# Mikubill/sketch2img

Measured on AMD Instinct MI355X. Metric: sketch-guided images/sec whole-node, SD1.5 512px 50-step DDIM, higher is better.
Workload: dtype fp16

## Files before the change

include/skg.h:

```cpp
#ifndef SKG_H_
#define SKG_H_

#include <stddef.h>
#include <stdint.h>

#ifdef __cplusplus
extern "C" {
#endif

#define SKG_OK 0
#define SKG_E_BADARG (-1)
#define SKG_E_UNSUPPORTED (-2)
#define SKG_E_LAUNCH (-3)

#define SKG_ABI_VERSION 6
int skg_abi_version(void);
const char* skg_last_error(void);

#define SKG_EPI_RELU 1u
#define SKG_EPI_OUT_F32 2u
#define SKG_EPI_GEGLU 4u
#define SKG_EPI_BIAS_ROWS 8u

int skg_gemm_f16(const void* A, int lda, const void* B, int ldb, void* C, void* C_lo, int ldc, int M, int N, int K,
                 const void* bias, const void* residual, const void* residual_lo, int ldr, float alpha, unsigned flags,
                 float* gn_partial, int HW, int groups, void* stream);

int skg_set_workspace(void* ws, size_t bytes, void* stream);

int skg_gemm_variant(int M, int N, int K, int Cin, int mode);

#define SKG_CONV_S1 0
#define SKG_CONV_S2 1
#define SKG_CONV_UP2 2
#define SKG_CONV_S2T 3
#define SKG_CONV_S2A 4
int skg_conv3x3_f16(const void* X, int ldx, const void* Wp, void* Y, void* Y_lo, int ldy, int rows, int IH, int IW,
                    int Cin, int Cout, int mode, const void* bias, const void* residual, const void* residual_lo, int ldr,
                    float alpha, unsigned flags, float* gn_partial, int groups, void* stream);

size_t skg_groupnorm_scratch_floats(int rows, int groups);
int skg_groupnorm_stats(const void* X, int ldx, int rows, int HW, int C, int groups, float eps,
                        float* stats, float* partial, void* stream);
int skg_groupnorm_fwd(const void* X, const void* X_lo, int ldx, void* Y, void* Y_lo, int ldy, int rows, int HW, int C, int groups,
                      float eps, const void* gamma, const void* beta, int silu, float* stats, float* partial, void* stream);
// ... 180 lines not shown
```

sketch2img_amd/_lib.py:

```python
from __future__ import annotations

import ctypes
import os

import torch

_HERE = os.path.dirname(os.path.abspath(__file__))
LIB_PATH = os.environ.get("SKG_LIB") or os.path.join(_HERE, "libskg.so")

ABI_VERSION = 6

SIGNATURES = {
    "skg_abi_version": ("i", ""),
    "skg_last_error": ("s", ""),
    "skg_gemm_f16": ("i", "pipippiiiipppifupiip"),
    "skg_conv3x3_up2_f16": ("i", "pipppiiiiiiipp"),
    "skg_conv3x3_sc_f16": ("i", "pipiipppiiiiiipupip"),
    "skg_conv4x4s2_f16": ("i", "pippiiiiiipp"),
    "skg_conv3x3_wino_v_bytes": ("z", "iiii"),
    "skg_conv3x3_wino_f16": ("i", "pippppiiiiiipppiup"),
    "skg_groupnorm_wino_fwd": ("i", "pipiiiiifppipp"),
    "skg_gemm_f16_rows": ("i", "pipipiiiipiip"),
    "skg_gemm_gn_fused": ("i", "iiiiiii"),
    "skg_gemm_f16_geglu_keep": ("i", "pipipipiiiipp"),
    "skg_ff_block_f16": ("i", "ppippiiiippfppppppippiipiip"),
    "skg_xattn_block_f16": ("i", "ppippiiiiiippfpppfpppipip"),
    "skg_gemm_variant": ("i", "iiiii"),
    "skg_set_workspace": ("i", "pzp"),
    "skg_conv3x3_f16": ("i", "pipppiiiiiiipppifupip"),
    "skg_groupnorm_scratch_floats": ("z", "ii"),
    "skg_groupnorm_stats": ("i", "piiiiifppp"),
    "skg_groupnorm_fwd": ("i", "ppippiiiiifppippp"),
    "skg_groupnorm_from_partial": ("i", "ppippiiiiiifppippipiip"),
    "skg_groupnorm_apply": ("i", "ppipiiiiipppip"),
    "skg_groupnorm_bwd": ("i", "pipipipiiiiipppipp"),
    "skg_layernorm_fwd": ("i", "ppipiiippfpp"),
    "skg_layernorm_bwd": ("i", "pipipipiiippp"),
    "skg_geglu_fwd": ("i", "pipiiiip"),
    "skg_geglu_bwd": ("i", "pipipiiiip"),
    "skg_attn_fwd": ("i", "pipipipipiiiiiifup"),
    "skg_attn_bwd_delta": ("i", "pipipiiiip"),
    "skg_attn_bwd_dq": ("i", "pipipipipippppiiiiiiifp"),
# ... 94 lines not shown
```

sketch2img_amd/csrc/gemm.hip:

```cpp
#include "gemm_params.h"
#include <mutex>
#include <vector>

namespace {

constexpr int BM = 128;
constexpr int BK = 32;
constexpr int PITCH = 40;

template <int BN, int MODE>
__global__ __launch_bounds__(256) void gemm_kernel(const GemmParams p) {
  constexpr int WN = BN / 2;
  constexpr int NT = WN / 16;
  constexpr int MT = 4;
  constexpr int BPT = BN / 64;
  __shared__ __attribute__((aligned(16))) half_t As[2][BM * PITCH];
  __shared__ __attribute__((aligned(16))) half_t Bs[2][BN * PITCH];

  const int tid = threadIdx.x;
  const int lane = tid & 63;
  const int wave = tid >> 6;
  const int wm = wave >> 1, wn = wave & 1;
  const int g = lane >> 4, l16 = lane & 15;
  const int m0 = blockIdx.y * BM;
// ... 266 lines not shown
#ifdef SKG_LAB
    q.C = (void*)16;
    if (skg_gemm9_eligible(q, mode)) return 9320;
    q.C = nullptr;
#endif
    if (const int bn8 = skg_gemm8_tile_n(q, mode)) return 8000 + bn8;
#ifdef SKG_LAB
    q.C = (void*)16;
    if (skg_gemmk_eligible(q, mode)) return 9160;
#endif
  }
  const int v2 = skg_gemm2_tile_n(M, N, K, Cin, mode, ws_query_bytes());
  return v2 ? 2000 + v2 : 1000 + (use_wide(M, N) ? 128 : 64);
}

extern "C" int skg_gemm_f16_geglu_keep(const void* A, int lda, const void* B, int ldb, void* Y, int ldy, void* H,
                                       int ldh, int M, int N, int K, const void* bias, void* stream) {
  SKG_REQUIRE(A && B && Y && H && M > 0 && N > 0 && K > 0 && K % 64 == 0 && N % 16 == 0);
  SKG_REQUIRE(lda % 8 == 0 && ldb % 8 == 0 && ldy % 8 == 0 && ldh % 8 == 0 && lda >= K && ldb >= K && ldy >= N / 2 && ldh >= N);
  SKG_REQUIRE(skg_aligned(A, 16) && skg_aligned(B, 16) && skg_aligned(Y, 16) && skg_aligned(H, 16));
  SKG_REQUIRE(!bias || skg_aligned(bias, 8));
  GemmParams p{};
  p.A = (const half_t*)A; p.lda = lda; p.B = (const half_t*)B; p.ldb = ldb; p.C = Y; p.ldc = ldy;
  p.bias = (const half_t*)bias; p.M = M; p.N = N; p.K = K; p.alpha = 1.f; p.flags = SKG_EPI_GEGLU;
  p.aux = (half_t*)H; p.ldaux = ldh;
  ws_attach(p, (hipStream_t)stream);
  return launch<MODE_DIRECT>(p, (hipStream_t)stream);
}

extern "C" int skg_gemm_gn_fused(int M, int N, int K, int Cin, int mode, int HW, int groups) {
// ... 227 lines not shown
```

sketch2img_amd/csrc/gemm2.hip:

```cpp
#include "gemm_params.h"
#include <stdlib.h>

namespace {

constexpr int BK = 64;
constexpr unsigned OOB = 0x80000000u;

typedef __attribute__((address_space(3))) void* lds_ptr_t;

__device__ __forceinline__ void dma16(__amdgpu_buffer_rsrc_t rsrc, half_t* lds_wave_base, unsigned voff,
                                      unsigned soff) {
  __builtin_amdgcn_raw_ptr_buffer_load_lds(rsrc, (lds_ptr_t)lds_wave_base, 16, voff, soff, 0, 0);
}

template <int MASK, int N>
__device__ __forceinline__ void sgb() {
  if constexpr (N > 0) __builtin_amdgcn_sched_group_barrier(MASK, N, 0);
}
constexpr int SGB_MFMA = 0x008, SGB_VMEM = 0x010, SGB_DSREAD = 0x100;
template <int NT, int R, int V>
__device__ __forceinline__ void sched_group() {
  if constexpr (NT > 0) {
    sgb<SGB_MFMA, 1>();
    if constexpr (R > 0) {
// ... 82 lines not shown
  if (p.flags & SKG_EPI_RELU) {
    v[0] = fmaxf(v[0], 0.f); v[1] = fmaxf(v[1], 0.f); v[2] = fmaxf(v[2], 0.f); v[3] = fmaxf(v[3], 0.f);
  }
  if (p.flags & SKG_EPI_OUT_F32) {
    *reinterpret_cast<float4_t*>(reinterpret_cast<float*>(p.C) + m * p.ldc + n) = v;
  } else {
    half4_t o = {(half_t)v[0], (half_t)v[1], (half_t)v[2], (half_t)v[3]};
    st_half4(reinterpret_cast<half_t*>(p.C) + m * p.ldc + n, o);
    if (p.c_lo) {
      half4_t l = {(half_t)(v[0] - (float)o[0]), (half_t)(v[1] - (float)o[1]), (half_t)(v[2] - (float)o[2]), (half_t)(v[3] - (float)o[3])};
      st_half4(p.c_lo + m * p.ldc + n, l);
    }
  }
}

template <int BM, int BN, int WGM, int WGN, int MODE, int NS, bool GNS, bool HILO, bool FIX, bool BROWS = false>
__device__ __forceinline__ void gemm2_body(const GemmParams& p, int tiles_n, int nwg, unsigned a_bytes, unsigned b_bytes,
                                           unsigned a_shift, int kt_per_split, float* __restrict__ ws) {
  constexpr int NW = WGM * WGN;
  constexpr int NTHR = NW * 64;
  constexpr int WM = BM / WGM;
  constexpr int WN = BN / WGN;
  constexpr int NT = WN / 16;
  constexpr int MT = WM / 16;
  constexpr int ACH = BM / 8 / NW;
  constexpr int BCH = BN / 8 / NW;
  static_assert(BM % (8 * NW) == 0 && BN % (8 * NW) == 0 && WM % 16 == 0 && WN % 16 == 0, "tile shape");
  constexpr int STAGE = (BM + BN) * BK;
  constexpr bool AFFINE = (MODE == MODE_DIRECT || MODE == MODE_S1 || MODE == MODE_S2 || MODE == MODE_S2A);
  __shared__ __attribute__((aligned(16))) half_t smem[NS * STAGE + 2 * BN];

  const int tid = threadIdx.x;
  const int lane = tid & 63;
  const int wave = __builtin_amdgcn_readfirstlane(tid >> 6);
  const int wm = wave / WGN, wn = wave - wm * WGN;
  const int g = lane >> 4, l16 = lane & 15;

  const __amdgpu_buffer_rsrc_t rA =
      __builtin_amdgcn_make_buffer_rsrc((void*)((const char*)p.A - a_shift), 0, a_bytes, 0x00020000);
  const __amdgpu_buffer_rsrc_t rB = __builtin_amdgcn_make_buffer_rsrc((void*)p.B, 0, b_bytes, 0x00020000);
  const __amdgpu_buffer_rsrc_t rA2 = __builtin_amdgcn_make_buffer_rsrc(
      (void*)(p.A2 ? p.A2 : p.A), 0, p.A2 ? ((unsigned)(p.M - 1) * (unsigned)p.lda2 + (unsigned)p.K2) * 2u : 0u, 0x00020000);
  const int KT1 = (MODE == MODE_S1 && p.K2) ? (p.K - p.K2) / BK : (1 << 30);

  for (int vb = blockIdx.x; vb < nwg; vb += gridDim.x) {
// ... 80 lines not shown
      } else {
        a_voff[j] = ok ? 0u : OOB;
        a_oy[j] = oy; a_ox[j] = ox;
        a_img[j] = img * (unsigned)p.lda * 2u + pk + a_shift;
      }
    }
  }
  unsigned b_voff[BCH];
#pragma unroll
  for (int j = 0; j < BCH; ++j) {
    const int r = (j * NW + wave) * 8 + lr;
    const unsigned pk = (unsigned)(lq ^ ((r >> 1) & 7)) * 16u;
    const int n = n0 + r;
    b_voff[j] = n < p.N ? ((unsigned)n + (p.up2 == 5 ? (unsigned)(ph * p.N) : 0u)) * (unsigned)p.ldb * 2u + pk : OOB;
  }

  const bool tap_minor = (p.flags & 0x1000u) != 0;
  struct DmaStep { unsigned va[ACH]; unsigned vb[BCH]; unsigned soa, sob; bool second; };
  auto dma_prepare = [&](int kt, bool live) {
    DmaStep d;
    d.second = false;
    if (MODE == MODE_S1 && kt >= KT1) {
      d.second = true;
#pragma unroll
      for (int j = 0; j < ACH; ++j) {
        const int r = (j * NW + wave) * 8 + lr;
        const unsigned pk = (unsigned)(lq ^ ((r >> 1) & 7)) * 16u;
        d.va[j] = (live && m0 + r < p.M) ? (unsigned)(m0 + r) * (unsigned)p.lda2 * 2u + pk : OOB;
      }
#pragma unroll
// ... 154 lines not shown
#ifdef SKG_LAB
    if (!(p.flags & 0x2000u))
#endif
    sched_plan<MT, NT, ND>();
  };

  const int kt_begin = split * kt_per_split;
  const int KT = min(p.K / BK, kt_begin + kt_per_split);
  float bias_r = 0.f;
  if constexpr (!BROWS) {
    const half_t* bias_t = p.bias;
    if constexpr (MODE != MODE_DIRECT) bias_t += __builtin_amdgcn_readfirstlane(smp0) * p.bias_pitch;
    bias_r = (tid < BN && p.bias && n0 + tid < p.N) ? (float)bias_t[n0 + tid] : 0.f;
  }
  SKG_PH(1);
  {
    const DmaStep d0 = dma_prepare(kt_begin, true);
#pragma unroll
    for (int i = 0; i < ND; ++i) dma_one(d0, 0, i);
  }
  if constexpr (NS == 2) {
    for (int kt = kt_begin; kt < KT; kt += 2) {
      asm volatile("s_waitcnt vmcnt(0)" ::: "memory");
      lds_barrier();
      step(kt + 1, 1, 0, KT);
      if (kt + 1 < KT) {
        asm volatile("s_waitcnt vmcnt(0)" ::: "memory");
        lds_barrier();
        step(kt + 2, 0, 1, KT);
      }
    }
  } else {
    static_assert(NS >= 3 && (NS - 2) * ND <= 63, "counted wait");
#pragma unroll
    for (int s = 1; s < NS - 1; ++s) {
      const DmaStep d1 = dma_prepare(kt_begin + s, kt_begin + s < KT);
#pragma unroll
      for (int i = 0; i < ND; ++i) dma_one(d1, s, i);
    }
    asm volatile("s_waitcnt vmcnt(0)" ::: "memory");
    for (int kt = kt_begin; kt < KT; kt += NS) {
#pragma unroll
      for (int s = 0; s < NS; ++s) {
        if (kt + s < KT) {
          asm volatile("s_waitcnt vmcnt(%0)" ::"n"((NS - 2) * ND) : "memory");
          lds_barrier();
          step(kt + s + NS - 1, (s + NS - 1) % NS, s, KT);
        }
      }
    }
  }
  asm volatile("s_waitcnt vmcnt(0)" ::: "memory");

  SKG_PH(2);
#ifdef SKG_PHASES
  if ((tid & 63) == 0 && vb < (1 << 15)) g_phase[vb][12 + (tid >> 6)] = __builtin_readcyclecounter();
#endif
  const bool stream_out = p.flags & 0x800u;
  const bool relu = p.flags & SKG_EPI_RELU;
  const bool f32out = p.flags & SKG_EPI_OUT_F32;
  if (ws) {
    float* slab = ws + (size_t)split * p.M * p.N;
#pragma unroll
    for (int i = 0; i < MT; ++i) {
      const int m = m0 + wm * WM + i * 16 + l16;
// ... 146 lines not shown
        const int nch = p.gn_hw >> 7, b = m0 / p.gn_hw, chunk = (m0 - b * p.gn_hw) >> 7;
        p.gn_partial[(((size_t)b * nch + chunk) * p.gn_groups + n0 / cpg + gi) * 2 + qq] = t;
      }
    }
  };
  if (staged && !p.res && !HILO && !BROWS) {
    constexpr int OPH = BN + 8;
    constexpr int HROWS = 128;
    constexpr int HSLABS = BM / HROWS;
    constexpr int PPR = BN / 8;
    constexpr int TPR2 = NTHR / 64;
    constexpr int IT2 = PPR / TPR2;
    constexpr int RPT = HROWS / 64;
    static_assert(HROWS * OPH * 2 <= 2 * STAGE * 2 && NTHR % 64 == 0 && PPR % TPR2 == 0, "fp16 staging slab");
    half_t* const hst = smem;
    float* const bias_s = reinterpret_cast<float*>(smem + NS * STAGE);
    const int er = tid / TPR2, ec = (tid % TPR2) * 8;
    const bool geglu = p.flags & SKG_EPI_GEGLU;
    if (tid < BN) bias_s[tid] = bias_r;
    half_t* const crow0 = reinterpret_cast<half_t*>(p.C) + (size_t)(m0 + er) * p.ldc + n0 + ec;
#pragma unroll
    for (int sl = 0; sl < HSLABS; ++sl) {
      lds_barrier();
      if (sl == 0) SKG_PH(8);
      if (WM < HROWS || wm == sl) {
#pragma unroll
        for (int j = 0; j < NT; ++j) {
          const float4_t b4 = *reinterpret_cast<const float4_t*>(&bias_s[wn * WN + j * 16 + g * 4]) * p.alpha;
#pragma unroll
          for (int i = 0; i < MT; ++i) acc[i][j] = acc[i][j] * p.alpha + b4;
        }
// ... 101 lines not shown
    }
    if (gn) gn_fold();
    SKG_PH(4);
    continue;
  }
  if (staged) {
    constexpr int OPF = BN + 4;
    constexpr int SROWS = 64;
    constexpr int SLABS = BM / SROWS;
    static_assert(SROWS * OPF * 4 <= 2 * STAGE * 2, "staging slab must fit in the pipeline stages");
    constexpr int PPR = BN / 8;
    constexpr int TPR = NTHR / SROWS;
    constexpr int ITER = PPR / TPR;
    static_assert(NTHR % SROWS == 0 && PPR % TPR == 0, "piece loop must have a compile-time trip count");
    float* const stg = reinterpret_cast<float*>(smem);
    float* const bias_s = reinterpret_cast<float*>(smem + NS * STAGE);
    const int er = tid / TPR, ec = (tid % TPR) * 8;
    if (tid < BN) bias_s[tid] = bias_r;
    constexpr bool RES_UP_FRONT = SLABS * ITER <= 10;
    half8_t rv[SLABS][ITER];
    const half_t* const rrow0 = p.res ? p.res + (size_t)(m0 + er) * p.ldr + n0 + ec : nullptr;
    auto load_res = [&](int sl) {
      const bool rowok = p.res && m0 + sl * SROWS + er < p.M;
#pragma unroll
      for (int k = 0; k < ITER; ++k)
        rv[sl][k] = (rowok && n0 + ec + k * TPR * 8 < p.N)
                        ? ld_half8(rrow0 + (size_t)sl * SROWS * p.ldr + k * TPR * 8) : zero_half8();
    };
    if (RES_UP_FRONT) {
#pragma unroll
      for (int sl = 0; sl < SLABS; ++sl) load_res(sl);
// ... 121 lines not shown
      }
      if (relu) {
        v[0] = fmaxf(v[0], 0.f); v[1] = fmaxf(v[1], 0.f); v[2] = fmaxf(v[2], 0.f); v[3] = fmaxf(v[3], 0.f);
      }
      if (f32out) {
        *reinterpret_cast<float4_t*>(reinterpret_cast<float*>(p.C) + (size_t)m * p.ldc + n) = v;
      } else {
        half4_t o = {(half_t)v[0], (half_t)v[1], (half_t)v[2], (half_t)v[3]};
        st_half4(reinterpret_cast<half_t*>(p.C) + (size_t)m * p.ldc + n, o);
      }
    }
  }
  }
}

template <int BM, int BN, int WGM, int WGN, int MODE, int NS = 2, bool GNS = false, bool HILO = false, bool BROWS = false>
__global__ __launch_bounds__(WGM * WGN * 64, (NS * (BM + BN) * BK * 2 + 8 * BN <= 80 * 1024) ? 2 : 1) void gemm2_kernel(const GemmParams p, int tiles_n, int nwg,
                                                                  unsigned a_bytes, unsigned b_bytes,
                                                                  unsigned a_shift, int kt_per_split,
                                                                  float* __restrict__ ws) {
  gemm2_body<BM, BN, WGM, WGN, MODE, NS, GNS, HILO, false, BROWS>(p, tiles_n, nwg, a_bytes, b_bytes, a_shift, kt_per_split, ws);
}
#ifdef SKG_LAB
template <int BM, int BN, int WGM, int WGN, int MODE>
__global__ __launch_bounds__(WGM * WGN * 64, (2 * (BM + BN) * BK * 2 + 8 * BN <= 80 * 1024) ? 2 : 1) void gemm2_splitk_kernel(const GemmParams p, int tiles_n, int nwg,
                                                                  unsigned a_bytes, unsigned b_bytes,
                                                                  unsigned a_shift, int kt_per_split,
                                                                  float* __restrict__ ws) {
  gemm2_body<BM, BN, WGM, WGN, MODE, 2, false, false, true>(p, tiles_n, nwg, a_bytes, b_bytes, a_shift, kt_per_split, ws);
}
#endif

__global__ __launch_bounds__(256) void splitk_reduce_kernel(const GemmParams p, const float* __restrict__ ws,
                                                            int splits) {
  const int N4 = p.N >> 2;
  const size_t total = (size_t)p.M * N4;
// ... 86 lines not shown

inline bool gn_fusable(const GemmParams& p, int mode) {
  if (!p.gn_partial || p.gn_groups <= 0 || p.gn_hw <= 0 || !eligible(p, mode)) return false;
  if (p.flags & (SKG_EPI_OUT_F32 | SKG_EPI_GEGLU)) return false;
  const bool hilo = p.c_lo || p.res_lo;
  TileCfg t = pick_tile(p.M, p.N, p.K);
  if (hilo && t.bm == 256) t = TileCfg{128, 160};
  if (t.bm != 128 || t.bn != 160) return false;
  if (p.M % 128 != 0 || p.N % 160 != 0 || p.gn_hw % 128 != 0 || p.M % p.gn_hw != 0 || p.N % p.gn_groups != 0) return false;
  const int cpg = p.N / p.gn_groups;
  if ((cpg & 1) || 160 % cpg != 0) return false;
  if (p.ldc % 8 != 0 || (reinterpret_cast<uintptr_t>(p.C) & 15) != 0) return false;
  if (p.res && (p.ldr % 8 != 0 || (reinterpret_cast<uintptr_t>(p.res) & 15) != 0)) return false;
  const long ntiles = (long)(p.M / 128) * (p.N / 160);
  return pick_splits(ntiles, p.K / BK, (size_t)p.M * p.N * 4, p.ws, p.ws_bytes) == 1;
}

template <int BM, int BN, int WGM, int WGN, int MODE>
void launch_cfg(const GemmParams& p_in, hipStream_t st) {
  GemmParams p = p_in;
  const size_t out_bytes = (size_t)p.M * ((p.flags & SKG_EPI_GEGLU) ? p.N / 2 : p.N) * ((p.flags & SKG_EPI_OUT_F32) ? 4 : 2);
  static const bool tap_major = getenv("SKG_TAP_MAJOR") != nullptr;
  if (MODE != MODE_DIRECT && !tap_major) p.flags |= 0x1000u;
#ifdef SKG_LAB
  if (MODE != MODE_DIRECT && getenv("SKG_GLUE_PROBE")) p.flags |= 0x2000u;
#endif
  static const char* smb = getenv("SKG_STREAM_MB");
  if (out_bytes >= (smb ? (size_t)atoi(smb) << 20 : STREAM_OUT_BYTES)) p.flags |= 0x800u;
#ifdef SKG_LAB
  static const int direct_epi = getenv("SKG_DIRECT_EPI") ? atoi(getenv("SKG_DIRECT_EPI")) : 0;
  const bool direct_ok = direct_epi && !(p.flags & (SKG_EPI_GEGLU | SKG_EPI_OUT_F32)) && !p.c_lo && !p.res_lo && !p.gn_partial && !p.up2 &&
                         !p.seg_rows && !p.ntaps && !p.bias_pitch && p.N % BN == 0 && p.ldc % 8 == 0 && skg_aligned(p.C, 16) &&
                         (!p.res || (p.ldr % 8 == 0 && skg_aligned(p.res, 16))) && (!p.bias || skg_aligned(p.bias, 16)) &&
                         (direct_epi == 1 || p.K <= 640);
#else
  constexpr bool direct_ok = false;
#endif
  const int tiles_n = skg_cdiv(p.N, BN);
  const int ntiles = skg_cdiv(p.M, BM) * tiles_n * (p.up2 == 5 ? 4 : 1);
  unsigned long long a, b, s;
  operand_bytes(p, MODE, a, b, s);
  const int KT = p.K / BK;
  int splits = (BM == 128 && !(p.flags & SKG_EPI_GEGLU) && !p.up2 && !p.seg_rows) ? pick_splits(ntiles, KT, (size_t)p.M * p.N * 4, p.ws, p.ws_bytes) : 1;
  if (p.wino) splits = p.wino;
  constexpr int NTHR = WGM * WGN * 64;
  if (BM == 128 && BN == 160 && splits == 1 && gn_fusable(p, MODE)) p.flags |= SKG_FLAG_GN_STATS;
  if (p.bias_pitch && (p.gn_hw % BM != 0 || (p.flags & SKG_EPI_OUT_F32) || p.ldc % 8 != 0 || !skg_aligned(p.C, 16) || (p.res && (p.ldr % 8 != 0 || !skg_aligned(p.res, 16)))))
    p.flags |= SKG_FLAG_BIAS_PER_ROW;
  if (direct_ok && splits == 1) p.flags |= 0x10000u;
  const int ns_eff = splits > 1 ? skg_cdiv(KT, skg_cdiv(KT, splits)) : 1;
  const int G = (8 % ns_eff == 0) ? 8 / ns_eff : 0;
  if (G >= 2 && ntiles % G == 0 && p.up2 != 5) {
    static const bool off = getenv("SKG_NO_XGRID") != nullptr;
    const int tiles_m = ntiles / tiles_n;
    const double a_mb = (double)p.M * (MODE == MODE_DIRECT ? p.K : p.Cin) * 2.0, w_mb = (double)p.N * p.K * 2.0;
    int best = 1;
    double cost = a_mb + G * w_mb;
    for (int gn = 2; gn <= G; gn *= 2) {
      if (tiles_n % gn != 0 || tiles_m % (G / gn) != 0) continue;
      const double c = gn * a_mb + (G / gn) * w_mb;
      if (c < 0.9 * cost) { cost = c; best = gn; }
    }
    static const char* force_gn = getenv("SKG_XGRID_GN");
// ... 9 lines not shown
#ifdef SKG_LAB
    if constexpr (BM == 128) {
      const bool self = getenv("SKG_SPLITK_SELF") != nullptr;
      if (p.ws_cnt && self && (size_t)ntiles * 4 <= SKG_WS_TICKET_BYTES && p.N % 4 == 0) {
        hipLaunchKernelGGL((gemm2_splitk_kernel<BM, BN, WGM, WGN, MODE>), dim3(ntiles * ns), dim3(NTHR), 0, st, p, tiles_n, ntiles * ns,
                           (unsigned)a, (unsigned)b, (unsigned)s, per, p.ws);
        return;
      }
    }
#endif
    bool deep = false;
    if constexpr (BM == 128 && BN == 160 && (MODE == MODE_DIRECT || MODE == MODE_S1)) {
      const int sns = split_tuning().ns;
      if (ntiles * ns <= 256 && per >= 4 && sns >= 3) {
        deep = true;
        if (sns >= 4)
          hipLaunchKernelGGL((gemm2_kernel<BM, BN, WGM, WGN, MODE, 4, false, false>), dim3(ntiles * ns), dim3(NTHR), 0, st, p, tiles_n, ntiles * ns,
                             (unsigned)a, (unsigned)b, (unsigned)s, per, p.ws);
        else
          hipLaunchKernelGGL((gemm2_kernel<BM, BN, WGM, WGN, MODE, 3, false, false>), dim3(ntiles * ns), dim3(NTHR), 0, st, p, tiles_n, ntiles * ns,
                             (unsigned)a, (unsigned)b, (unsigned)s, per, p.ws);
      }
    }
    if (!deep)
      hipLaunchKernelGGL((gemm2_kernel<BM, BN, WGM, WGN, MODE>), dim3(persistent_grid(ntiles * ns, NTHR)), dim3(NTHR),
                         0, st, p, tiles_n, ntiles * ns, (unsigned)a, (unsigned)b, (unsigned)s, per, p.ws);
    if (p.wino) return;
    size_t blocks = ((size_t)p.M * (p.N / 4) + 255) / 256;
    hipLaunchKernelGGL(splitk_reduce_kernel, dim3((unsigned)(blocks > 2048 ? 2048 : blocks)), dim3(256), 0, st, p,
                       (const float*)p.ws, ns);
    return;
// ... 18 lines not shown
#define G2_LAUNCH(NS_, GNS_, HILO_)                                                                                            \
  hipLaunchKernelGGL((gemm2_kernel<BM, BN, WGM, WGN, MODE, NS_, GNS_, HILO_>), dim3(ntiles), dim3(NTHR), 0, st, p, tiles_n, ntiles, \
                     (unsigned)a, (unsigned)b, (unsigned)s, KT, (float*)nullptr)
  if constexpr (BM == 128 && (BN == 160 || BN == 64) && (MODE == MODE_DIRECT || MODE == MODE_S1)) {
    static const bool off = getenv("SKG_NO_NS3") != nullptr;
#ifdef SKG_LAB
    if (!off && !gns && !hilo && ntiles <= 256) {
      const char* e = getenv("SKG_NS");
      const int ns = e ? atoi(e) : 0;
      if (ns == 4 && KT >= 5) { G2_LAUNCH(4, false, false); return; }
      if constexpr (BN == 64) {
        if (ns == 6 && KT >= 7) { G2_LAUNCH(6, false, false); return; }
      }
    }
#endif
    if (!off && KT >= 4 && (BN == 64 || ntiles <= 256)) {
      if constexpr (BN == 160) {
        if (gns) {
          if (hilo) G2_LAUNCH(3, true, true); else G2_LAUNCH(3, true, false);
          return;
        }
      }
      if (hilo) G2_LAUNCH(3, false, true); else G2_LAUNCH(3, false, false);
      return;
    }
  }
#ifdef SKG_PHASES
  static const char* solo = getenv("SKG_SOLO");
  if (solo) {
    hipLaunchKernelGGL((gemm2_kernel<BM, BN, WGM, WGN, MODE>), dim3(ntiles), dim3(NTHR), 48 * 1024, st,
                       p, tiles_n, ntiles, (unsigned)a, (unsigned)b, (unsigned)s, KT, (float*)nullptr);
// ... 10 lines not shown
    }
  }
  if constexpr (BM == 128 && BN == 160) {
    if (gns) { G2_LAUNCH(2, true, false); return; }
  }
#undef G2_LAUNCH
  hipLaunchKernelGGL((gemm2_kernel<BM, BN, WGM, WGN, MODE>), dim3(persistent_grid(ntiles, NTHR)), dim3(NTHR), 0, st,
                     p, tiles_n, ntiles, (unsigned)a, (unsigned)b, (unsigned)s, KT, (float*)nullptr);
}

template <int MODE>
void launch_mode(const GemmParams& p, hipStream_t st) {
  TileCfg t = pick_tile(p.M, p.N, p.K);
  if (t.bm == 256 && (p.c_lo || p.res_lo || p.up2 || p.seg_rows || p.bias_pitch)) t = TileCfg{128, 160};
  if (p.wino) t = p.N % 160 == 0 ? TileCfg{128, 160} : p.N % 128 == 0 ? TileCfg{128, 128} : TileCfg{128, 64};
  if (t.bm == 256) launch_cfg<256, 320, 2, 4, MODE>(p, st);
  else if (t.bn == 160) {
    launch_cfg<128, 160, 2, 2, MODE>(p, st);
  }
  else if (t.bn == 128) launch_cfg<128, 128, 2, 2, MODE>(p, st);
  else launch_cfg<128, 64, 2, 2, MODE>(p, st);
}

}

int skg_gemm2_tile_n(int M, int N, int K, int Cin, int mode, size_t ws_bytes) {
  if (K % BK != 0 || M < 1 || (mode != MODE_DIRECT && Cin % BK != 0)) return 0;
  const TileCfg t = pick_tile(M, N, K);
  const int KT = K / BK;
  const long ntiles = (long)skg_cdiv(M, t.bm) * skg_cdiv(N, t.bn);
  const int splits = t.bm == 128 ? pick_splits(ntiles, KT, (size_t)M * N * 4, ws_bytes ? (const float*)1 : nullptr, ws_bytes) : 1;
  bool three = t.bm == 128 && (t.bn == 160 || t.bn == 64) && (mode == MODE_DIRECT || mode == MODE_S1) &&
               !getenv("SKG_NO_NS3") && KT >= 4 && (t.bn == 64 || ntiles <= 256) && splits == 1;
  if (splits > 1 && t.bm == 128 && t.bn == 160 && (mode == MODE_DIRECT || mode == MODE_S1)) {
    const int per = skg_cdiv(KT, splits), ns = skg_cdiv(KT, per);
    three = ntiles * ns <= 256 && per >= 4 && split_tuning().ns >= 3;
  }
  return t.bn + (three ? 10000 : 0);
}

bool skg_gemm2_fuses_gn(const GemmParams& p, int mode) { return gn_fusable(p, mode); }

void skg_splitk_reduce_launch(const GemmParams& p, const float* ws, int splits, hipStream_t st) {
  size_t blocks = ((size_t)p.M * (p.N / 4) + 255) / 256;
  hipLaunchKernelGGL(splitk_reduce_kernel, dim3((unsigned)(blocks > 2048 ? 2048 : blocks)), dim3(256), 0, st, p, ws, splits);
}

bool skg_gemm2_try_launch(const GemmParams& p, int mode, hipStream_t st) {
  if (!eligible(p, mode)) return false;
  if (p.wino &&
      (mode != MODE_DIRECT || p.wino != 16 || (p.K / BK) % 16 != 0 || !p.ws || (size_t)16 * p.M * p.N * 4 > p.ws_bytes || p.gn_partial ||
       p.seg_rows || p.up2 || p.aux || (p.flags & (SKG_EPI_GEGLU | SKG_EPI_OUT_F32))))
    return false;
  if (p.seg_rows &&
      (mode != MODE_DIRECT || p.res || p.gn_partial || p.c_lo || p.res_lo || p.aux || (p.flags & (SKG_EPI_GEGLU | SKG_EPI_OUT_F32)) ||
       p.ldc % 8 != 0 || (reinterpret_cast<uintptr_t>(p.C) & 15) != 0))
// ... 33 lines not shown
```

sketch2img_amd/csrc/gemm_params.h:

```cpp
#pragma once
#include "common.h"

enum { MODE_DIRECT = 0, MODE_S1 = 1, MODE_S2 = 2, MODE_UP2 = 3, MODE_S2T = 4, MODE_S2A = 5 };

struct GemmParams {
  const half_t* A; int lda;
  const half_t* B; int ldb;
  void* C; int ldc;
  const half_t* bias;
  const half_t* res; int ldr;
  int M, N, K;
  float alpha; unsigned flags;
  int IH, IW, OH, OW, Cin;
  float* gn_partial; int gn_hw, gn_groups;
  half_t* aux; int ldaux;
  const half_t* res_lo; half_t* c_lo;
  int ntaps; unsigned tapmap; int up2;
  int a_wrap;
  int seg_rows, seg_stride;
  const half_t* A2; int lda2, K2;
  int wino;
  float* ws; size_t ws_bytes;
  unsigned* ws_cnt;
  int bias_pitch;
};
constexpr unsigned SKG_FLAG_GN_STATS = 0x8000u;
constexpr unsigned SKG_FLAG_BIAS_PER_ROW = 0x20000u;

bool skg_gemm2_try_launch(const GemmParams& p, int mode, hipStream_t st);
constexpr size_t SKG_WS_TICKET_BYTES = 16 << 10;
int skg_gemm2_tile_n(int M, int N, int K, int Cin, int mode, size_t ws_bytes);
bool skg_gemmws_eligible(const GemmParams& p, int mode);
bool skg_gemmws_try_launch(const GemmParams& p, int mode, hipStream_t st);
bool skg_gemm8_eligible(const GemmParams& p, int mode);
int skg_gemm8_tile_n(const GemmParams& p, int mode);
bool skg_gemm8_try_launch(const GemmParams& p, int mode, hipStream_t st);
bool skg_gemm9_eligible(const GemmParams& p, int mode);
bool skg_gemm9_try_launch(const GemmParams& p, int mode, hipStream_t st);
bool skg_gemmk_eligible(const GemmParams& p, int mode);
bool skg_gemmk_try_launch(const GemmParams& p, int mode, hipStream_t st);
void skg_splitk_reduce_launch(const GemmParams& p, const float* ws, int splits, hipStream_t st);
bool skg_gemm8_fuses_gn(const GemmParams& p, int mode);
bool skg_gemm2_fuses_gn(const GemmParams& p, int mode);
void skg_wino_in_launch(const half_t* X, int ldx, half_t* V, int rows, int IH, int IW, int Cin, hipStream_t st);
void skg_wino_out_launch(const GemmParams& p, const float* slabs, int IH, int IW, hipStream_t st);
void skg_gn_partial_launch(const half_t* X, int ldx, int rows, int HW, int C, int groups, int nch, float* partial,
// ... 2 lines not shown
```

Measured before the change: 6.136.

## Add halo-slab implicit-GEMM path for stride-1 3x3 convs

Adds a slab variant of the 128x160 gemm2 kernel for stride-1 3x3 convolutions. It loads a haloed input slab (rows plus a one-pixel border) into LDS once per channel block and reuses it across all nine taps, instead of re-gathering the A operand for each tap. Slab loads are double-buffered, and weight tiles go through a three-stage ring. The path is enabled by default at level 2 and selected by shape and split heuristics, with an env var and API to change the level. The cost is more LDS per block, more precomputed address registers and much more kernel complexity, with a risk of lower occupancy.

New measurement: 6.196, median of 6. No clear change (+1.0%).

```diff
diff --git a/include/skg.h b/include/skg.h
--- a/include/skg.h
+++ b/include/skg.h
@@ -29,6 +29,9 @@
 int skg_set_workspace(void* ws, size_t bytes, void* stream);
 
 int skg_gemm_variant(int M, int N, int K, int Cin, int mode);
+
+int skg_conv_slab_set(int level);
+int skg_conv_slab_takes(int rows, int IH, int IW, int Cin, int Cout, int K2, int pair);
 
 #define SKG_CONV_S1 0
 #define SKG_CONV_S2 1
diff --git a/sketch2img_amd/_lib.py b/sketch2img_amd/_lib.py
--- a/sketch2img_amd/_lib.py
+++ b/sketch2img_amd/_lib.py
@@ -26,6 +26,8 @@
     "skg_ff_block_f16": ("i", "ppippiiiippfppppppippiipiip"),
     "skg_xattn_block_f16": ("i", "ppippiiiiiippfpppfpppipip"),
     "skg_gemm_variant": ("i", "iiiii"),
+    "skg_conv_slab_set": ("i", "i"),
+    "skg_conv_slab_takes": ("i", "iiiiiii"),
     "skg_set_workspace": ("i", "pzp"),
     "skg_conv3x3_f16": ("i", "pipppiiiiiiipppifupip"),
     "skg_groupnorm_scratch_floats": ("z", "ii"),
diff --git a/sketch2img_amd/csrc/gemm.hip b/sketch2img_amd/csrc/gemm.hip
--- a/sketch2img_amd/csrc/gemm.hip
+++ b/sketch2img_amd/csrc/gemm.hip
@@ -304,6 +304,21 @@
   return v2 ? 2000 + v2 : 1000 + (use_wide(M, N) ? 128 : 64);
 }
 
+extern "C" int skg_conv_slab_set(int level) { return skg_gemm2_conv_slab_set(level); }
+
+extern "C" int skg_conv_slab_takes(int rows, int IH, int IW, int Cin, int Cout, int K2, int pair) {
+  if (rows <= 0 || IH <= 0 || IW <= 0 || Cin <= 0 || Cout <= 0 || K2 < 0) return 0;
+  static float dummy;
+  GemmParams q{};
+  q.lda = Cin; q.ldb = 9 * Cin + K2; q.ldc = Cout; q.N = Cout; q.K = 9 * Cin + K2; q.Cin = Cin; q.K2 = K2;
+  q.IH = q.OH = IH; q.IW = q.OW = IW; q.M = rows * IH * IW; q.gn_hw = IH * IW;
+  q.c_lo = pair ? reinterpret_cast<half_t*>(&dummy) : nullptr;
+  const size_t wsb = ws_query_bytes();
+  q.ws = wsb ? &dummy : nullptr; q.ws_bytes = wsb;
+  if (skg_gemm8_eligible(q, MODE_S1)) return 0;
+  return skg_gemm2_slab_width(q, MODE_S1) ? 1 : 0;
+}
+
 extern "C" int skg_gemm_f16_geglu_keep(const void* A, int lda, const void* B, int ldb, void* Y, int ldy, void* H,
                                        int ldh, int M, int N, int K, const void* bias, void* stream) {
   SKG_REQUIRE(A && B && Y && H && M > 0 && N > 0 && K > 0 && K % 64 == 0 && N % 16 == 0);
diff --git a/sketch2img_amd/csrc/gemm2.hip b/sketch2img_amd/csrc/gemm2.hip
--- a/sketch2img_amd/csrc/gemm2.hip
+++ b/sketch2img_amd/csrc/gemm2.hip
@@ -1,5 +1,6 @@
 #include "gemm_params.h"
 #include <stdlib.h>
+#include <atomic>
 
 namespace {
 
@@ -120,7 +121,12 @@
   }
 }
 
-template <int BM, int BN, int WGM, int WGN, int MODE, int NS, bool GNS, bool HILO, bool FIX, bool BROWS = false>
+template <int V> struct IntC { static constexpr int value = V; };
+template <int I, int N, class F>
+__device__ __forceinline__ void static_for(F&& f) {
+  if constexpr (I < N) { f(IntC<I>{}); static_for<I + 1, N>(f); }
+}
+template <int BM, int BN, int WGM, int WGN, int MODE, int NS, bool GNS, bool HILO, bool FIX, bool BROWS = false, int SLABW = 0>
 __device__ __forceinline__ void gemm2_body(const GemmParams& p, int tiles_n, int nwg, unsigned a_bytes, unsigned b_bytes,
                                            unsigned a_shift, int kt_per_split, float* __restrict__ ws) {
   constexpr int NW = WGM * WGN;
@@ -134,7 +140,14 @@
   static_assert(BM % (8 * NW) == 0 && BN % (8 * NW) == 0 && WM % 16 == 0 && WN % 16 == 0, "tile shape");
   constexpr int STAGE = (BM + BN) * BK;
   constexpr bool AFFINE = (MODE == MODE_DIRECT || MODE == MODE_S1 || MODE == MODE_S2 || MODE == MODE_S2A);
-  __shared__ __attribute__((aligned(16))) half_t smem[NS * STAGE + 2 * BN];
+  constexpr bool SLAB = SLABW != 0;
+  constexpr int SLABH = 36 * 8 * BK;
+  constexpr int WST = BN * BK;
+  constexpr int SLAB_W0 = 2 * SLABH;
+  constexpr int LDS_H = SLAB ? SLAB_W0 + 3 * WST : NS * STAGE;
+  static_assert(!SLAB || (NS == 3 && BM == 128 && BN == 160 && NW == 4 && MODE == MODE_S1 && !FIX && !BROWS && LDS_H >= NS * STAGE &&
+                          (SLABW == 16 || SLABW == 32 || SLABW == 64)), "halo-slab form");
+  __shared__ __attribute__((aligned(16))) half_t smem[LDS_H + 2 * BN];
 
   const int tid = threadIdx.x;
   const int lane = tid & 63;
@@ -245,6 +258,34 @@
     const int n = n0 + r;
     b_voff[j] = n < p.N ? ((unsigned)n + (p.up2 == 5 ? (unsigned)(ph * p.N) : 0u)) * (unsigned)p.ldb * 2u + pk : OOB;
   }
+  unsigned s_voff[9];
+  int a_tab[16][2];
+  int bw_ad[NT][2];
+  if constexpr (SLAB) {
+    constexpr int PW = SLABW + 2, NPIX = (128 / SLABW + 2) * PW;
+    const int hw = p.IH * p.IW;
+    const int smp = m0 / hw, y0 = (m0 - smp * hw) / SLABW;
+#pragma unroll
+    for (int t = 0; t < 9; ++t) {
+      const int s = (t * NW + wave) * 8 + lr;
+      const int sy = s / PW, sx = s - sy * PW;
+      const int iy = y0 - 1 + sy, ix = sx - 1;
+      const bool ok = s < NPIX && iy >= 0 && iy < p.IH && ix >= 0 && ix < p.IW;
+      s_voff[t] = ok ? ((unsigned)(smp * hw + (y0 + sy) * p.IW + sx) * (unsigned)p.lda) * 2u + (unsigned)(lq ^ ((s >> 1) & 7)) * 16u : OOB;
+    }
+    const int S_w = wm * (WM / SLABW) * PW;
+#pragma unroll
+    for (int bb = 0; bb < 16; ++bb)
+#pragma unroll
+      for (int ks = 0; ks < 2; ++ks)
+        a_tab[bb][ks] = ((S_w + l16) * BK + (((ks * 4 + g) ^ (((bb + S_w + l16) >> 1) & 7)) << 3)) * 2;
+#pragma unroll
+    for (int j = 0; j < NT; ++j) {
+      const int row = wn * WN + j * 16 + l16;
+#pragma unroll
+      for (int ks = 0; ks < 2; ++ks) bw_ad[j][ks] = SLAB_W0 + row * BK + (((ks * 4 + g) ^ ((row >> 1) & 7)) << 3);
+    }
+  }
 
   const bool tap_minor = (p.flags & 0x1000u) != 0;
   struct DmaStep { unsigned va[ACH]; unsigned vb[BCH]; unsigned soa, sob; bool second; };
@@ -429,13 +470,96 @@
     bias_r = (tid < BN && p.bias && n0 + tid < p.N) ? (float)bias_t[n0 + tid] : 0.f;
   }
   SKG_PH(1);
+  int kt0 = kt_begin;
+  if constexpr (SLAB) {
+    const int KT3 = min(KT, KT1);
+    if (kt_begin < KT3) {
+      const int cb0 = kt_begin / 9, t0 = kt_begin - 9 * cb0, cbl = (KT3 - 1) / 9;
+#pragma unroll
+      for (int t = 0; t < 9; ++t)
+        dma16(rA, &smem[(cb0 & 1) * SLABH + (t * NW + wave) * 8 * BK], s_voff[t], (unsigned)cb0 * (BK * 2u));
+#pragma unroll
+      for (int t = 0; t < 8; ++t)
+        if (t < t0)
+          dma16(rA, &smem[((cb0 + 1) & 1) * SLABH + (t * NW + wave) * 8 * BK], cb0 < cbl ? s_voff[t] : OOB, (unsigned)(cb0 + 1) * (BK * 2u));
+#pragma unroll
+      for (int s = 0; s < 2; ++s) {
+        const int kt = kt_begin + s, cq = kt / 9, ti = kt - 9 * cq;
+#pragma unroll
+        for (int j = 0; j < BCH; ++j)
+          dma16(rB, &smem[SLAB_W0 + (kt % 3) * WST + (j * NW + wave) * 8 * BK], kt < KT3 ? b_voff[j] : OOB,
+                (unsigned)(ti * p.Cin + cq * BK) * 2u);
+      }
+      if (cb0 & 1) {
+#pragma unroll
+        for (int bb = 0; bb < 16; ++bb) { a_tab[bb][0] += SLABH * 2; a_tab[bb][1] += SLABH * 2; }
+      }
+      asm volatile("s_waitcnt vmcnt(0)" ::: "memory");
+      for (int cb = cb0; cb <= cbl; ++cb) {
+        const bool nxt = cb < cbl;
+        half_t* const fill = &smem[((cb + 1) & 1) * SLABH + wave * 8 * BK];
+        static_for<0, 9>([&](auto tc) {
+          constexpr int TAP = decltype(tc)::value;
+          const int kt = 9 * cb + TAP;
+          if (kt >= kt_begin && kt < KT3) {
+            asm volatile("s_waitcnt vmcnt(%0)" ::"n"(BCH) : "memory");
+            lds_barrier();
+            constexpr int CS = TAP % 3, IS = (TAP + 2) % 3;
+            constexpr int TI2 = (TAP + 2) % 9, CQ2 = (TAP + 2) / 9;
+            const bool wlive = kt + 2 < KT3;
+            const unsigned sob = (unsigned)(TI2 * p.Cin + (cb + CQ2) * BK) * 2u;
+            auto dma_slab = [&](int i) {
+              if (i == 0) dma16(rA, fill + TAP * NW * 8 * BK, nxt ? s_voff[TAP] : OOB, (unsigned)(cb + 1) * (BK * 2u));
+              else dma16(rB, &smem[SLAB_W0 + IS * WST + ((i - 1) * NW + wave) * 8 * BK], wlive ? b_voff[i - 1] : OOB, sob);
+            };
+            half8_t xf[2][MT], wf[2][NT];
+            auto rd = [&](int idx) {
+              auto xa = [&](int i, int ks) {
+                const int sc = ((i * 16) / SLABW + TAP / 3) * (SLABW + 2) + (i * 16) % SLABW + TAP % 3;
+                return reinterpret_cast<const half_t*>(reinterpret_cast<const char*>(smem) + a_tab[sc & 15][ks] + sc * (BK * 2));
+              };
+              if (idx < NT) wf[0][idx] = ld_half8(smem + CS * WST + bw_ad[idx][0]);
+              else if (idx < NT + MT) xf[0][idx - NT] = ld_half8(xa(idx - NT, 0));
+              else if (idx < 2 * NT + MT) wf[1][idx - NT - MT] = ld_half8(smem + CS * WST + bw_ad[idx - NT - MT][1]);
+              else xf[1][idx - 2 * NT - MT] = ld_half8(xa(idx - 2 * NT - MT, 1));
+            };
+            int ri = 0, di = 0;
+#pragma unroll
+            for (int r = 0; r < plan_initial<MT, NT>(); ++r) rd(ri++);
+#pragma unroll
+            for (int gq = 0; gq < 2 * MT; ++gq) {
+#pragma unroll
+              for (int r = 0; r < plan_reads<MT, NT>(gq); ++r) rd(ri++);
+#pragma unroll
+              for (int v = 0; v < plan_vmem<MT, NT>(gq, BCH + 1); ++v) dma_slab(di++);
+            }
+#pragma unroll
+            for (int ks = 0; ks < 2; ++ks)
+#pragma unroll
+              for (int i = 0; i < MT; ++i)
+#pragma unroll
+                for (int j = 0; j < NT; ++j)
+                  acc[i][j] = __builtin_amdgcn_mfma_f32_16x16x32_f16(wf[ks][j], xf[ks][i], acc[i][j], 0, 0, 0);
+            sched_plan<MT, NT, BCH + 1>();
+          }
+        });
+        const int flip = (cb & 1) ? -SLABH * 2 : SLABH * 2;
+#pragma unroll
+        for (int bb = 0; bb < 16; ++bb) { a_tab[bb][0] += flip; a_tab[bb][1] += flip; }
+      }
+      asm volatile("s_waitcnt vmcnt(0)" ::: "memory");
+      kt0 = KT3;
+      if (kt0 < KT) lds_barrier();
+    }
+  }
+  if (!SLAB || kt0 < KT) {
   {
-    const DmaStep d0 = dma_prepare(kt_begin, true);
+    const DmaStep d0 = dma_prepare(kt0, true);
 #pragma unroll
     for (int i = 0; i < ND; ++i) dma_one(d0, 0, i);
   }
   if constexpr (NS == 2) {
-    for (int kt = kt_begin; kt < KT; kt += 2) {
+    for (int kt = kt0; kt < KT; kt += 2) {
       asm volatile("s_waitcnt vmcnt(0)" ::: "memory");
       lds_barrier();
       step(kt + 1, 1, 0, KT);
@@ -449,12 +573,12 @@
     static_assert(NS >= 3 && (NS - 2) * ND <= 63, "counted wait");
 #pragma unroll
     for (int s = 1; s < NS - 1; ++s) {
-      const DmaStep d1 = dma_prepare(kt_begin + s, kt_begin + s < KT);
+      const DmaStep d1 = dma_prepare(kt0 + s, kt0 + s < KT);
 #pragma unroll
       for (int i = 0; i < ND; ++i) dma_one(d1, s, i);
     }
     asm volatile("s_waitcnt vmcnt(0)" ::: "memory");
-    for (int kt = kt_begin; kt < KT; kt += NS) {
+    for (int kt = kt0; kt < KT; kt += NS) {
 #pragma unroll
       for (int s = 0; s < NS; ++s) {
         if (kt + s < KT) {
@@ -464,6 +588,7 @@
         }
       }
     }
+  }
   }
   asm volatile("s_waitcnt vmcnt(0)" ::: "memory");
 
@@ -640,7 +765,7 @@
     constexpr int RPT = HROWS / 64;
     static_assert(HROWS * OPH * 2 <= 2 * STAGE * 2 && NTHR % 64 == 0 && PPR % TPR2 == 0, "fp16 staging slab");
     half_t* const hst = smem;
-    float* const bias_s = reinterpret_cast<float*>(smem + NS * STAGE);
+    float* const bias_s = reinterpret_cast<float*>(smem + LDS_H);
     const int er = tid / TPR2, ec = (tid % TPR2) * 8;
     const bool geglu = p.flags & SKG_EPI_GEGLU;
     if (tid < BN) bias_s[tid] = bias_r;
@@ -772,7 +897,7 @@
     constexpr int ITER = PPR / TPR;
     static_assert(NTHR % SROWS == 0 && PPR % TPR == 0, "piece loop must have a compile-time trip count");
     float* const stg = reinterpret_cast<float*>(smem);
-    float* const bias_s = reinterpret_cast<float*>(smem + NS * STAGE);
+    float* const bias_s = reinterpret_cast<float*>(smem + LDS_H);
     const int er = tid / TPR, ec = (tid % TPR) * 8;
     if (tid < BN) bias_s[tid] = bias_r;
     constexpr bool RES_UP_FRONT = SLABS * ITER <= 10;
@@ -924,12 +1049,12 @@
   }
 }
 
-template <int BM, int BN, int WGM, int WGN, int MODE, int NS = 2, bool GNS = false, bool HILO = false, bool BROWS = false>
+template <int BM, int BN, int WGM, int WGN, int MODE, int NS = 2, bool GNS = false, bool HILO = false, bool BROWS = false, int SLABW = 0>
 __global__ __launch_bounds__(WGM * WGN * 64, (NS * (BM + BN) * BK * 2 + 8 * BN <= 80 * 1024) ? 2 : 1) void gemm2_kernel(const GemmParams p, int tiles_n, int nwg,
                                                                   unsigned a_bytes, unsigned b_bytes,
                                                                   unsigned a_shift, int kt_per_split,
                                                                   float* __restrict__ ws) {
-  gemm2_body<BM, BN, WGM, WGN, MODE, NS, GNS, HILO, false, BROWS>(p, tiles_n, nwg, a_bytes, b_bytes, a_shift, kt_per_split, ws);
+  gemm2_body<BM, BN, WGM, WGN, MODE, NS, GNS, HILO, false, BROWS, SLABW>(p, tiles_n, nwg, a_bytes, b_bytes, a_shift, kt_per_split, ws);
 }
 #ifdef SKG_LAB
 template <int BM, int BN, int WGM, int WGN, int MODE>
@@ -1046,6 +1171,45 @@
   if (p.res && (p.ldr % 8 != 0 || (reinterpret_cast<uintptr_t>(p.res) & 15) != 0)) return false;
   const long ntiles = (long)(p.M / 128) * (p.N / 160);
   return pick_splits(ntiles, p.K / BK, (size_t)p.M * p.N * 4, p.ws, p.ws_bytes) == 1;
+}
+
+std::atomic<int> g_conv_slab{-1};
+constexpr int CONV_SLAB_DEFAULT = 2;
+inline int conv_slab_level() {
+  int v = g_conv_slab.load(std::memory_order_relaxed);
+  if (v < 0) {
+    const char* e = getenv("SKG_CONV_SLAB");
+    v = e ? atoi(e) : CONV_SLAB_DEFAULT;
+    v = v < 0 ? 0 : v > 4 ? 4 : v;
+    g_conv_slab.store(v, std::memory_order_relaxed);
+  }
+  return v;
+}
+inline bool slab_shape_ok(const GemmParams& p, int mode) {
+  static const bool other_walk = getenv("SKG_TAP_MAJOR") != nullptr || getenv("SKG_NO_NS3") != nullptr;
+  return mode == MODE_S1 && !other_walk && !p.ntaps && !p.up2 && !p.seg_rows && !p.wino && !p.a_wrap && p.Cin % BK == 0 &&
+         (p.IW == 16 || p.IW == 32 || p.IW == 64) && p.OH == p.IH && p.OW == p.IW && (p.IH * p.IW) % 128 == 0 &&
+         p.M % (p.IH * p.IW) == 0 && p.K == 9 * p.Cin + p.K2;
+}
+inline bool slab_forces_tile(const GemmParams& p, int mode) {
+  return mode == MODE_S1 && conv_slab_level() >= 4 && p.N % 160 == 0 && slab_shape_ok(p, mode);
+}
+inline bool slab_pick(int level, long ntiles, int KT, int& splits) {
+  if (level >= 2 && splits == 2 && ntiles == 256) splits = 1;
+  if (splits == 1) return KT >= 4 && (ntiles <= 256 || (level >= 3 && ntiles == 512));
+  const int per = skg_cdiv(KT, splits), ns = skg_cdiv(KT, per);
+  return ntiles * ns <= 256 && per >= 4 && split_tuning().ns == 3;
+}
+
+template <int BM, int BN, int WGM, int WGN, bool GNS, bool HILO>
+void launch_slab(int w, const GemmParams& p, int nwg, hipStream_t st, int tiles_n, unsigned a, unsigned b, unsigned s, int per, float* ws) {
+#define G2_SLAB(W_)                                                                                                                    \
+  hipLaunchKernelGGL((gemm2_kernel<BM, BN, WGM, WGN, MODE_S1, 3, GNS, HILO, false, W_>), dim3(nwg), dim3(WGM * WGN * 64), 0, st, p, tiles_n, \
+                     nwg, a, b, s, per, ws)
+  if (w == 16) G2_SLAB(16);
+  else if (w == 32) G2_SLAB(32);
+  else G2_SLAB(64);
+#undef G2_SLAB
 }
 
 template <int BM, int BN, int WGM, int WGN, int MODE>
@@ -1076,9 +1240,15 @@
   int splits = (BM == 128 && !(p.flags & SKG_EPI_GEGLU) && !p.up2 && !p.seg_rows) ? pick_splits(ntiles, KT, (size_t)p.M * p.N * 4, p.ws, p.ws_bytes) : 1;
   if (p.wino) splits = p.wino;
   constexpr int NTHR = WGM * WGN * 64;
+  const bool bias_per_row = p.bias_pitch && (p.gn_hw % BM != 0 || (p.flags & SKG_EPI_OUT_F32) || p.ldc % 8 != 0 || !skg_aligned(p.C, 16) ||
+                                             (p.res && (p.ldr % 8 != 0 || !skg_aligned(p.res, 16))));
+  int slabw = 0;
+  if constexpr (BM == 128 && BN == 160 && MODE == MODE_S1) {
+    const int level = conv_slab_level();
+    if (level && !bias_per_row && slab_shape_ok(p, MODE) && slab_pick(level, ntiles, KT, splits)) slabw = p.IW;
+  }
   if (BM == 128 && BN == 160 && splits == 1 && gn_fusable(p, MODE)) p.flags |= SKG_FLAG_GN_STATS;
-  if (p.bias_pitch && (p.gn_hw % BM != 0 || (p.flags & SKG_EPI_OUT_F32) || p.ldc % 8 != 0 || !skg_aligned(p.C, 16) || (p.res && (p.ldr % 8 != 0 || !skg_aligned(p.res, 16)))))
-    p.flags |= SKG_FLAG_BIAS_PER_ROW;
+  if (bias_per_row) p.flags |= SKG_FLAG_BIAS_PER_ROW;
   if (direct_ok && splits == 1) p.flags |= 0x10000u;
   const int ns_eff = splits > 1 ? skg_cdiv(KT, skg_cdiv(KT, splits)) : 1;
   const int G = (8 % ns_eff == 0) ? 8 / ns_eff : 0;
@@ -1118,7 +1288,9 @@
       const int sns = split_tuning().ns;
       if (ntiles * ns <= 256 && per >= 4 && sns >= 3) {
         deep = true;
-        if (sns >= 4)
+        if (slabw)
+          launch_slab<BM, BN, WGM, WGN, false, false>(slabw, p, ntiles * ns, st, tiles_n, (unsigned)a, (unsigned)b, (unsigned)s, per, p.ws);
+        else if (sns >= 4)
           hipLaunchKernelGGL((gemm2_kernel<BM, BN, WGM, WGN, MODE, 4, false, false>), dim3(ntiles * ns), dim3(NTHR), 0, st, p, tiles_n, ntiles * ns,
                              (unsigned)a, (unsigned)b, (unsigned)s, per, p.ws);
         else
@@ -1167,7 +1339,19 @@
       }
     }
 #endif
-    if (!off && KT >= 4 && (BN == 64 || ntiles <= 256)) {
+    if (!off && KT >= 4 && (BN == 64 || ntiles <= 256 || slabw)) {
+      if constexpr (BN == 160 && MODE == MODE_S1) {
+        if (slabw) {
+          if (gns) {
+            if (hilo) launch_slab<BM, BN, WGM, WGN, true, true>(slabw, p, ntiles, st, tiles_n, (unsigned)a, (unsigned)b, (unsigned)s, KT, nullptr);
+            else launch_slab<BM, BN, WGM, WGN, true, false>(slabw, p, ntiles, st, tiles_n, (unsigned)a, (unsigned)b, (unsigned)s, KT, nullptr);
+          } else {
+            if (hilo) launch_slab<BM, BN, WGM, WGN, false, true>(slabw, p, ntiles, st, tiles_n, (unsigned)a, (unsigned)b, (unsigned)s, KT, nullptr);
+            else launch_slab<BM, BN, WGM, WGN, false, false>(slabw, p, ntiles, st, tiles_n, (unsigned)a, (unsigned)b, (unsigned)s, KT, nullptr);
+          }
+          return;
+        }
+      }
       if constexpr (BN == 160) {
         if (gns) {
           if (hilo) G2_LAUNCH(3, true, true); else G2_LAUNCH(3, true, false);
@@ -1208,6 +1392,7 @@
   TileCfg t = pick_tile(p.M, p.N, p.K);
   if (t.bm == 256 && (p.c_lo || p.res_lo || p.up2 || p.seg_rows || p.bias_pitch)) t = TileCfg{128, 160};
   if (p.wino) t = p.N % 160 == 0 ? TileCfg{128, 160} : p.N % 128 == 0 ? TileCfg{128, 128} : TileCfg{128, 64};
+  if (slab_forces_tile(p, MODE)) t = TileCfg{128, 160};
   if (t.bm == 256) launch_cfg<256, 320, 2, 4, MODE>(p, st);
   else if (t.bn == 160) {
     launch_cfg<128, 160, 2, 2, MODE>(p, st);
@@ -1234,6 +1419,24 @@
 }
 
 bool skg_gemm2_fuses_gn(const GemmParams& p, int mode) { return gn_fusable(p, mode); }
+
+int skg_gemm2_conv_slab_set(int level) {
+  const int prev = conv_slab_level();
+  g_conv_slab.store(level < 0 ? 0 : level > 4 ? 4 : level, std::memory_order_relaxed);
+  return prev;
+}
+
+int skg_gemm2_slab_width(const GemmParams& p, int mode) {
+  if (!eligible(p, mode) || mode != MODE_S1) return 0;
+  TileCfg t = pick_tile(p.M, p.N, p.K);
+  if (t.bm == 256 && (p.c_lo || p.res_lo || p.up2 || p.seg_rows || p.bias_pitch)) t = TileCfg{128, 160};
+  if (slab_forces_tile(p, mode)) t = TileCfg{128, 160};
+  const int level = conv_slab_level();
+  if (!level || t.bm != 128 || t.bn != 160 || !slab_shape_ok(p, mode) || (p.bias_pitch && p.gn_hw % 128 != 0)) return 0;
+  const int ntiles = skg_cdiv(p.M, 128) * skg_cdiv(p.N, 160), KT = p.K / BK;
+  int splits = pick_splits(ntiles, KT, (size_t)p.M * p.N * 4, p.ws, p.ws_bytes);
+  return slab_pick(level, ntiles, KT, splits) ? p.IW : 0;
+}
 
 void skg_splitk_reduce_launch(const GemmParams& p, const float* ws, int splits, hipStream_t st) {
   size_t blocks = ((size_t)p.M * (p.N / 4) + 255) / 256;
diff --git a/sketch2img_amd/csrc/gemm_params.h b/sketch2img_amd/csrc/gemm_params.h
--- a/sketch2img_amd/csrc/gemm_params.h
+++ b/sketch2img_amd/csrc/gemm_params.h
@@ -30,6 +30,8 @@
 bool skg_gemm2_try_launch(const GemmParams& p, int mode, hipStream_t st);
 constexpr size_t SKG_WS_TICKET_BYTES = 16 << 10;
 int skg_gemm2_tile_n(int M, int N, int K, int Cin, int mode, size_t ws_bytes);
+int skg_gemm2_conv_slab_set(int level);
+int skg_gemm2_slab_width(const GemmParams& p, int mode);
 bool skg_gemmws_eligible(const GemmParams& p, int mode);
 bool skg_gemmws_try_launch(const GemmParams& p, int mode, hipStream_t st);
 bool skg_gemm8_eligible(const GemmParams& p, int mode);
```
